# driskai/scenario_gym

Measured on AMD Instinct MI355X. Metric: entity-steps/sec (batched rollout), higher is better.
Workload: dtype f64

## Files before the change

### scenario_gym_amd/csrc/h_queue.hip

```cpp
#include "sgym_host.hpp"

using namespace sgh;

enum { Q_HOST_RING = 16 };
int sgh::check_queue(sg_handle *h)
{
    for (; h->q_count > 0; --h->q_count) {
        const unsigned *w = h->q_host + (size_t)((h->q_head - h->q_count + Q_HOST_RING) % Q_HOST_RING) * sg::Q_STATE_WORDS;
        const unsigned code = w[sg::Q_ERR];
        if (code == 0 || h->q_failed) continue;
        static const char *what[] = {"", "a rollout wavefront waited for the controller pre-pass", "a rollout wavefront waited for the previous chunk of its block",
                                     "the controller pre-pass waited for a buffer of the table ring"};
        h->q_failed = true;
        h->queue_mode = 0;
        snprintf(h->q_msg, sizeof h->q_msg, "sg_rollout: the persistent table launch gave up (%s longer than SG_QUEUE_TIMEOUT_MS; %u work items had finished): "
                                            "the state of the batch is undefined -- sg_reset / sg_upload before the next call", what[code < 4 ? code : 0],
                 w[sg::Q_ITEMS_DONE]);
    }
    return h->q_failed ? fail(h, SG_ERR_HIP, "%s", h->q_msg) : SG_OK;
}
void sgh::forget_queue_failure(sg_handle *h)
{
    h->q_count = 0;
    h->q_failed = false;
// ... 194 lines not shown
}

int sgh::launch_table(sg_handle *h, const LaunchPlan &pl, int n_steps, int force, const double *d_actions, size_t *ev_next)
{
    if (pl.schedule == SCHED_TAB_DUMMY) {
        if (!h->d_tab[0]) {
            HIP_TRY(h, hipMalloc((void **)&h->d_tab[0], 64 * sizeof(double)));
            HIP_TRY(h, hipMalloc((void **)&h->d_tab[1], 64 * sizeof(double)));
            h->tab_bytes = 64 * sizeof(double);
            h->n_tab = 2;
            HIP_TRY(h, hipMemsetAsync(h->d_tab[0], 0, 64 * sizeof(double), h->stream));
        }
        return launch_main(h, pl, pl.fam, n_steps, 0, force, nullptr, h->d_tab[0], ev_next);
    }
    const bool no_overlap = !h->overlap;
    const size_t np = (size_t)h->p.n_ctl_pad, row = (size_t)sg::CT_PLANES * sg::CT_W * np;
    int ch = (int)std::min<size_t>((size_t)std::max(1, h->chunk_steps), std::max<size_t>(1, ((size_t)1 << 27) / row));
    ch = std::min(ch, n_steps);
    if (pl.rss_tab) ch = std::min(ch, std::max(1, h->rssq_steps));
    int rc = SG_QUEUE_FALLBACK;
    if (h->queue_mode && h->WV == 1 && !pl.riders && !no_overlap && np / 64 <= std::min((size_t)h->n_simd, slots_of(h, pl.rss_tab)) / 2 )
        rc = launch_queue(h, n_steps, force, d_actions, ch, ev_next, pl.rss_tab);
    if (rc != SG_QUEUE_FALLBACK) return rc;
    h->last_schedule = 1;
    const int NB = 2;
    const int ctl_slice = h->ctl_slice;
    if (ch > h->p.tab_steps || (size_t)(h->p.tab_steps + 1) * row * sizeof(double) > h->tab_bytes || NB > h->n_tab) {
        const int ts = std::max(ch, h->p.tab_steps);
        const size_t need = (size_t)(ts + 1) * row * sizeof(double);
        if (need > h->tab_bytes || NB > h->n_tab) {
            HIP_TRY(h, hipStreamSynchronize(h->stream));
// ... 27 lines not shown
        n = std::min(std::min(ch, c < 20 ? (2 * h->ctl_slice) << c : ch), n_steps - k0);
        ck0.push_back(k0);
        cn.push_back(n);
    }
    const int C = (int)cn.size();
    std::vector<hipEvent_t> ctl_done((size_t)C, nullptr), chunk_done((size_t)C, nullptr);
    int ctl_issued = 0;
    auto issue_ctl = [&](int upto) -> int {
        for (; ctl_issued <= upto && ctl_issued < C; ++ctl_issued) {
            const int c = ctl_issued, k0 = ck0[(size_t)c], n = cn[(size_t)c];
            double *tab = h->d_tab[c % NB];
            if (!no_overlap && c >= NB)
                HIP_TRY(h, hipStreamWaitEvent(cs, chunk_done[(size_t)(c - NB)], 0));
            for (int s0 = 0; s0 < n; s0 += ctl_slice)
                sgl::control(pl.ctl, cgrid, cs, h->p, h->cfg.timestep, std::min(ctl_slice, n - s0), c == 0 && s0 == 0, k0 + s0, d_actions,
                             tab, s0, pl.ctl_metrics);
            HIP_TRY(h, hipGetLastError());
            if (!no_overlap) {
                const int rc2 = get_event(h, (*ev_next)++, &ctl_done[(size_t)c]);
                if (rc2) return rc2;
                HIP_TRY(h, hipEventRecord(ctl_done[(size_t)c], cs));
            }
        }
        return SG_OK;
    };
    for (int c = 0; c < C; ++c) {
        if ((rc = issue_ctl(std::min(C - 1, c + NB - 1)))) return rc;
        const int b = c % NB;
        const sg::TabGroups tg = one_group(h, h->d_tab[b], cn[(size_t)c]);
        if (!no_overlap) HIP_TRY(h, hipStreamWaitEvent(h->stream, ctl_done[(size_t)c], 0));
        if ((rc = launch_main(h, pl, pl.fam, cn[(size_t)c], 0, force, nullptr, h->d_tab[b], ev_next, &tg))) return rc;
// ... 5 lines not shown
```

### scenario_gym_amd/csrc/h_slice.hip

```cpp
#include "sgym_host.hpp"

using namespace sgh;

static void launch_slice_kernels(sg_handle *h, const Params &ps, const sg::SliceArgs &sa, dim3 grid, const double *tab)
{
    note_slice(h, tab != nullptr);
    sgl::rollout_slice(h->G, grid, h->stream, ps, h->cfg.timestep, sa, tab);
}
static void launch_fixup_kernel(sg_handle *h, const Params &ps, const sg::SliceArgs &sa)
{
    sgl::replay_fixup(h->G, dim3((unsigned)(h->NE / 64)), h->stream, ps, sa, h->d_n_final);
}

struct SlicePlan { int S, len, SG; size_t bytes; };

static SlicePlan slice_plan(const sg_handle *h, int n_steps)
{
    const size_t nblk = h->NE / 64, R = (size_t)h->R, T1 = (size_t)n_steps + 1;
    const bool ctl = h->n_ctl > 0;
    SlicePlan pl{};
    pl.SG = (int)std::max<size_t>(1, 4096 / nblk);
    if (ctl && h->slice_mode == 2) pl.SG = std::min(pl.SG, 8);
    if (!ctl) {
        int S = (int)std::min<size_t>((size_t)pl.SG, (size_t)std::max(1, n_steps / (h->slice_mode == 2 ? 7 : 64)));
// ... 83 lines not shown
        HIP_TRY(h, hipEventRecord(e_reset, h->stream));
        HIP_TRY(h, hipStreamWaitEvent(h->ctl_stream, e_reset, 0));
    }
    HIP_TRY(h, hipMemsetAsync(sa.first_done, 0x7f, (size_t)R * S * sizeof(int), h->stream));
    HIP_TRY(h, hipMemsetAsync(sa.nev, 0, (size_t)R * S * sizeof(int), h->stream));
    const int n_clocks = (int)h->clock_t0.size();
    sgl::clock(dim3((unsigned)((n_clocks + 63) / 64)), h->stream, h->d_clock_t0, n_clocks, h->cfg.timestep, n_steps, const_cast<double *>(sa.tt));
    sa.mode = 0;
    const int ctl_len = std::max(1, env_int("SG_SLICE_CTL_STEPS", 2048));
    for (int s0 = 0; s0 < S; s0 += pl.SG) {
        const int ns = std::min(pl.SG, S - s0);
        if (ctl) {
            const int k0 = s0 * len, k1 = std::min(n_steps, (s0 + ns) * len);
            const dim3 cgrid((unsigned)(ps.n_ctl_pad / 64));
            for (int k = k0; k < k1; k += ctl_len)
                sgl::control(sgl::CTL_FAST, cgrid, h->ctl_stream, ps, h->cfg.timestep, std::min(ctl_len, k1 - k), k == 0, k, nullptr, h->d_slice_tab, k, 0);
            HIP_TRY(h, hipGetLastError());
            hipEvent_t e_c = nullptr;
            if ((rc = get_event(h, ev_next++, &e_c))) return rc;
            HIP_TRY(h, hipEventRecord(e_c, h->ctl_stream));
            HIP_TRY(h, hipStreamWaitEvent(h->stream, e_c, 0));
        }
        hipEvent_t e0 = nullptr, e1 = nullptr;
        if ((rc = get_event(h, ev_next, &e0)) || (rc = get_event(h, ev_next + 1, &e1))) return rc;
        HIP_TRY(h, hipEventRecord(e0, h->stream));
        sa.slice0 = s0;
        launch_slice_kernels(h, ps, sa, dim3((unsigned)nblk, (unsigned)ns), tab);
        HIP_TRY(h, hipGetLastError());
        HIP_TRY(h, hipEventRecord(e1, h->stream));
        h->launch_ev.push_back((int)ev_next);
        ++h->n_launches;
// ... 30 lines not shown
```

### scenario_gym_amd/csrc/k_ctl.hip

```cpp
#define SG_UNIT_CTL
#include "sgym_launch.hpp"

namespace sgl {
void control(int which, dim3 grid, hipStream_t s, const sg::Params &p, double timestep, int n_steps, int first, int k0,
             const double *actions, double *tab, int row0, int metrics)
{
    if (which == CTL_RIDERS) sg::control_kernel_riders<<<grid, dim3(64), 0, s>>>(p, timestep, n_steps, first, k0, actions, tab, row0, metrics);
    else if (which == CTL_FAST) sg::control_kernel_fast<<<grid, dim3(64), 0, s>>>(p, timestep, n_steps, first, k0, actions, tab, row0, metrics);
    else sg::control_kernel<<<grid, dim3(64), 0, s>>>(p, timestep, n_steps, first, k0, actions, tab, row0, metrics);
}
}
```

### scenario_gym_amd/csrc/sgym_control.hpp

```cpp
#pragma once

namespace sg {

struct CtlLds { double ctrl[9][64]; double seg[5][64]; };

template <bool FAST, bool RIDERS = false>
__device__ __forceinline__ void control_body_l(CtlLds &lds ,
                                               const unsigned qblock ,
                                               const Params &p, double timestep, int n_steps, int first, int k0,
                                               const double *actions , double *tab, int row0, int metrics)
{
    const int lane = threadIdx.x;
    const size_t q = (size_t)qblock * 64 + lane;
    const int ent_raw = p.ctl_ent[q];
    const bool active = ent_raw >= 0;
    const uint32_t ent = active ? (uint32_t)ent_raw : 0u;
    const uint32_t r = ent / (uint32_t)p.EP;
    const LanePtr st(p.stat + (size_t)(ent >> 6) * (ST_COUNT * 64), (ent & 63) * 8u);
    const LanePtr dy(p.dyn + (size_t)(ent >> 6) * ((size_t)p.FROWS * 64), (ent & 63) * 8u);
    const int64_t meta = fld<int64_t>(st, ST_META);
    const int kind = active ? (int)(meta & 0xff) : SG_KIND_NONE;
    const double min_t = fld(st, ST_MIN_T), bl = fld(st, ST_BL);
    const bool is_ego = active && (int)(ent - r * (uint32_t)p.EP) == p.sstat[r].ego;
#pragma unroll
    for (int c = 0; c < 9; ++c) lds.ctrl[c][lane] = fld(st, ST_CTRL + c);
    const size_t NP = (size_t)p.n_ctl_pad;
    double *cst = p.ctl_state + q;

    double pose[6], t, prev_t;
    double m_avg, m_max, m_t;
    bool present;
    CtrlState cs;
    if (first) {
        const sg_scenario_state &sd = p.sdyn[r];
        t = sd.t;
        prev_t = sd.prev_t;
        m_avg = sd.ego_avg_speed; m_max = sd.ego_max_speed; m_t = sd.avg_t;
        present = fld<uint64_t>(dy, SG_F_PRESENT) != 0;
#pragma unroll
        for (int c = 0; c < 6; ++c) pose[c] = fld(dy, SG_F_POSE + c);
        cs.speed = fld(dy, SG_F_CTRL + 0); cs.e_lon_prev = fld(dy, SG_F_CTRL + 1);
        cs.e_lat_prev = fld(dy, SG_F_CTRL + 2); cs.e_lon_int = fld(dy, SG_F_CTRL + 3);
    } else {
#pragma unroll
        for (int c = 0; c < 6; ++c) pose[c] = cst[(CS_POSE + c) * NP];
        present = cst[CS_PRESENT * NP] != 0.0;
        cs.speed = cst[(CS_CTRL + 0) * NP]; cs.e_lon_prev = cst[(CS_CTRL + 1) * NP];
        cs.e_lat_prev = cst[(CS_CTRL + 2) * NP]; cs.e_lon_int = cst[(CS_CTRL + 3) * NP];
        t = cst[CS_T * NP];
        prev_t = cst[CS_PREV_T * NP];
        m_avg = cst[(CS_METRIC + 0) * NP]; m_max = cst[(CS_METRIC + 1) * NP]; m_t = cst[(CS_METRIC + 2) * NP];
    }
    if (!active) present = false;

    Table T;
    {
        const double *kn = p.knots + fld<int64_t>(st, ST_KNOT_OFF) * 7;
        T.x = kn; T.xs = 7; T.y = kn + 1; T.ys = 7; T.cs = 1;
        T.n = active ? (int)(meta >> 32) : 0;
    }
    double seg_hi;
    int seg_cur;
    double sgr[5] = {0.0, 0.0, 0.0, 0.0, 0.0};
    auto seg_publish = [&](const Segment &S) {
        lds.seg[0][lane] = S.x_lo;
        lds.seg[1][lane] = S.ylo[0]; lds.seg[2][lane] = S.ylo[1];
// ... 63 lines not shown
            steer = __builtin_fmin(__builtin_fmax(steer, -max_steer), max_steer);
            const double dxs = speed0 * cos_h, dys = speed0 * sin_h;
            double tan_s = sg_tan_poly(steer, K);
            const bool steep = !(__builtin_fabs(steer) < 0.67434);
            if (sg_any(steep & active)) {
                double s2, c2;
                sg_sincos_core(steer, s2, c2, K);
                tan_s = steep ? s2 / c2 : tan_s;
            }
            const double hnum = speed0 * tan_s;
            const double dh = hnum == 0.0 ? hnum : rd_l.div(hnum);
            const double nx = pose[0] + dxs * dt, ny = pose[1] + dys * dt, nh = pose[3] + dh * dt;
            double nspeed = speed0 + accel * dt;
            nspeed = allow_rev == 0.0 ? __builtin_fmax(0.0, nspeed) : nspeed;
            nspeed = max_speed == max_speed ? __builtin_fmin(max_speed, nspeed) : nspeed;
            bool ok = rd.safe(d_lat) & rd.safe(d_lon) & (__builtin_fabs(steer) < 1.0e5) & (rd_l.safe(hnum) | (hnum == 0.0));
            double n_avg = m_avg, n_max = m_max, n_mt = m_t;
            if (metrics) {
                const RecipDiv rdt(dt), rnt(next_t);
                const double ax = nx - pose[0], ay = ny - pose[1];
                const double az = pose[2] - pose[2];
                const double speed = sg_norm3(rdt.div(ax), rdt.div(ay), 0.0);
                const double w = rnt.div(m_t);
                n_avg = m_avg + (1.0 - w) * (speed - m_avg);
                n_max = __builtin_fmax(speed, m_max);
                n_mt = next_t;
                ok = ok & (!is_ego | (rdt.safe(ax) & rdt.safe(ay) & rnt.safe(m_t) & (dt > 0.0) & (az == 0.0)));
            }
            if (sg_all(!active || ok)) {
                cs.e_lat_prev = e_lat; cs.e_lon_prev = e_lon; cs.e_lon_int = e_lon_I; cs.speed = nspeed;
                pose[0] = nx; pose[1] = ny; pose[3] = nh;
                if (is_ego) { m_avg = n_avg; m_max = n_max; m_t = n_mt; }
                prev_t = t;
                t = next_t;
                *reinterpret_cast<double4 *>(out + (size_t)k * CT_W) = make_double4(pose[0], pose[1], pose[3], cs.speed);
                *reinterpret_cast<double4 *>(out1 + (size_t)k * CT_W) = make_double4(cs.e_lon_prev, cs.e_lat_prev, cs.e_lon_int, 0.0);
                if (is_ego && metrics) *reinterpret_cast<double4 *>(out2 + (size_t)k * CT_W) = make_double4(m_avg, m_max, m_t, 0.0);
                continue;
            }
        }
        double act_a = 0.0, act_s = 0.0;
        if (kind == SG_KIND_AGENT_VEHICLE && actions) {
            const double *a = actions + ((size_t)(k0 + k) * p.R + r) * 2;
            act_a = a[0];
            act_s = a[1];
        }
        if (next_t > seg_hi) {
            Segment S;
            S.x_hi = seg_hi;
            S.cur = seg_cur;
            seg_advance(T, S, next_t);
            seg_publish(S);
// ... 21 lines not shown
            auto cp = [&](int q) -> double { return lds.ctrl[q][lane]; };
            if (kind == SG_KIND_AGENT_PID)
                pid_step(cs, cp, bl, state_dt, dt, tx, ty, sin_h, cos_h, np_, K);
            else
                vehicle_step(cs, cp, bl, dt, act_a, act_s, sin_h, cos_h, np_, K);
        } else if (active && min_t >= t) {
            npres = true;
            Segment S;
            S.cur = seg_cur;
            seg_load(T, S);
            sg_loads_done();
            const double dqs = next_t - S.x_lo;
#pragma unroll
            for (int c = 0; c < 6; ++c) np_[c] = S.sl[c] * dqs + S.ylo[c];
        }
        if (is_ego && npres && metrics) {
            double prev[6];
            if (!present) {
                own_position_extrap(T.x, T.n, t, prev);
                sg_loads_done();
            } else {
#pragma unroll
                for (int c = 0; c < 6; ++c) prev[c] = pose[c];
            }
            const double v0 = (np_[0] - prev[0]) / dt, v1 = (np_[1] - prev[1]) / dt, v2 = (np_[2] - prev[2]) / dt;
            const double speed = sg_norm3(v0, v1, v2);
            const double w = m_t / next_t;
            m_avg += (1.0 - w) * (speed - m_avg);
            m_t = next_t;
            m_max = __builtin_fmax(speed, m_max);
        }
        present = npres;
        if (npres) {
#pragma unroll
            for (int c = 0; c < 6; ++c) pose[c] = np_[c];
        }
        prev_t = t;
        t = next_t;
        *reinterpret_cast<double4 *>(out + (size_t)k * CT_W) = make_double4(pose[0], pose[1], pose[3], cs.speed);
        *reinterpret_cast<double4 *>(out1 + (size_t)k * CT_W) = make_double4(cs.e_lon_prev, cs.e_lat_prev, cs.e_lon_int, 0.0);
        if (is_ego && metrics) *reinterpret_cast<double4 *>(out2 + (size_t)k * CT_W) = make_double4(m_avg, m_max, m_t, 0.0);
        if (RIDERS) *reinterpret_cast<double4 *>(out2 + (size_t)k * CT_W) = make_double4(pose[2], pose[4], pose[5], present ? 1.0 : 0.0);
    }
#pragma unroll
    for (int c = 0; c < 6; ++c) cst[(CS_POSE + c) * NP] = pose[c];
    cst[CS_PRESENT * NP] = present ? 1.0 : 0.0;
    cst[(CS_CTRL + 0) * NP] = cs.speed; cst[(CS_CTRL + 1) * NP] = cs.e_lon_prev;
    cst[(CS_CTRL + 2) * NP] = cs.e_lat_prev; cst[(CS_CTRL + 3) * NP] = cs.e_lon_int;
    cst[CS_T * NP] = t;
    cst[CS_PREV_T * NP] = prev_t;
    cst[(CS_METRIC + 0) * NP] = m_avg; cst[(CS_METRIC + 1) * NP] = m_max; cst[(CS_METRIC + 2) * NP] = m_t;
}

template <bool FAST, bool RIDERS = false>
__device__ __forceinline__ void control_body(const Params &p, double timestep, int n_steps, int first, int k0,
                                             const double *actions , double *tab, int row0, int metrics)
{
    __shared__ CtlLds lds;
    control_body_l<FAST, RIDERS>(lds, blockIdx.x, p, timestep, n_steps, first, k0, actions, tab, row0, metrics);
}

#ifdef SG_UNIT_CTL
static __global__ __launch_bounds__(64, SG_CTL_WAVES) void control_kernel(Params p, double timestep, int n_steps, int first, int k0,
                                                     const double *actions , double *tab, int row0, int metrics)
{
    control_body<false>(p, timestep, n_steps, first, k0, actions, tab, row0, metrics);
}
#endif
#ifdef SG_UNIT_CTL
static __global__ __launch_bounds__(64, 2) void control_kernel_riders(Params p, double timestep, int n_steps, int first, int k0,
                                                               const double *actions , double *tab, int row0, int metrics)
{
    control_body<false, true>(p, timestep, n_steps, first, k0, actions, tab, row0, 0);
}
#endif
#ifdef SG_UNIT_CTL
static __global__ __launch_bounds__(64, 1) void control_kernel_fast(Params p, double timestep, int n_steps, int first, int k0,
                                                             const double *actions , double *tab, int row0, int metrics)
{
#ifdef SG_CTL_SETPRIO
    __builtin_amdgcn_s_setprio(3);
#endif
    control_body<true>(p, timestep, n_steps, first, k0, actions, tab, row0, metrics);
}
#endif

}
```

### scenario_gym_amd/csrc/sgym_core.hpp

```cpp
#pragma once

namespace sg {

enum {
    ST_BW = 0, ST_BL, ST_BCX, ST_BCY,
    ST_MIN_T, ST_MAX_T,
    ST_KNOT_OFF,
    ST_META,
    ST_ROUTE,
    ST_CTL,
    ST_CTRL,
    NCTRL_ROWS = 13,
    ST_COUNT = ST_CTRL + NCTRL_ROWS
};
constexpr uint32_t ROW = 512;

struct ScenStatic {
    double t0, length;
    int64_t grid_off;
    int32_t grid_n, ego;
};

struct RoadNet { double x0, y0, inv_cell; int32_t nx, ny; int64_t cell_base; };
struct RoadCand { int32_t poly; uint32_t edge_off; uint16_t n_edges; uint8_t ref_sel, ref_inside; };
// ... 54 lines not shown
    const double *noise_normals;
    long long noise_len;
    unsigned long long noise_seed;
    int ped_behaviour;
    int n_ped_models;
    const double *ped_models;
    const int32_t *model_of;
#ifdef SG_PHASE_TIMERS
    unsigned long long *phase_cycles;
#endif
};

enum { PM_BEHAVIOUR = 0, PM_SF = 1, PM_STD_LON = 13, PM_STD_LAT = 14, PM_W = 16 };
static_assert(sizeof(sg_social_force) == 12 * sizeof(double), "sg_social_force is twelve doubles");

enum { CT_X = 0, CT_Y, CT_H, CT_SPEED, CT_W = 4, CT_ELON = 0, CT_ELAT, CT_EINT, CT_MAVG = 0, CT_MMAX, CT_MT, CT_PLANES = 3 };
enum { CS_POSE = 0, CS_PRESENT = 6, CS_CTRL = 7, CS_T = 11, CS_PREV_T = 12, CS_METRIC = 13, CS_COUNT = 16 };

#define SG_GLOBAL __attribute__((address_space(1)))
struct LanePtr {
    SG_GLOBAL char *a[3];
    __device__ __forceinline__ LanePtr(const double *blk, uint32_t voff)
    {
        a[0] = (SG_GLOBAL char *)(reinterpret_cast<char *>(const_cast<double *>(blk)) + voff);
        a[1] = a[0] + 8 * ROW;
        a[2] = a[0] + 16 * ROW;
        asm("" : "+v"(a[1]), "+v"(a[2]));
    }
};
template <typename T = double>
__device__ __forceinline__ T fld(const LanePtr &lp, int f)
{
// ... 344 lines not shown
```

### scenario_gym_amd/csrc/sgym_hip.hip

```cpp
#include "sgym_host.hpp"

using namespace sgh;

static void note_kernel(sg_handle *h, const char *fmt, int a = 0, int b = 0) { snprintf(h->last_kernel, sizeof h->last_kernel, fmt, a, b); }
void sgh::note_wide(sg_handle *h) { note_kernel(h, "sg::wide_move_kernel + wide_commit_kernel + wide_collide_kernel + wide_finish_kernel"); }
void sgh::note_queue(sg_handle *h, bool rss)
{
    note_kernel(h, rss ? "sg::rollout_kernel_rss_tabq<%d>" : (h->planar ? "sg::rollout_kernel_tabq_planar<%d>" : "sg::rollout_kernel_tabq<%d>"), h->G);
}
void sgh::note_slice(sg_handle *h, bool tab) { note_kernel(h, tab ? "sg::rollout_kernel_slice_tab<%d>" : "sg::rollout_kernel_slice<%d>", h->G); }

static Fam pick_family(const sg_handle *h, bool rss, bool tab)
{
    const bool ped = h->has_ped, off_road = (h->cfg.terminal_mask & SG_TERM_EGO_OFF_ROAD) != 0;
    if (h->WV == 8) {
        if (!ped && off_road) return Fam::ROAD_W8;
        if (rss && !ped) return Fam::RSS_W8;
        return ped ? Fam::PED_W8 : Fam::PLAIN_W8;
    }
    if (ped && h->all_ped && h->G == 64 && crowd_road_ok(h) && crowd_allowed(h) && !rss) return Fam::CROWD;
    if (tab && ped && h->G == 64) return Fam::CROWD_RIDERS;
    if (ped && rss) return Fam::RSS_PED;
    if (rss && off_road) return Fam::RSS_ROAD;
    if (ped) return Fam::PED;
// ... 93 lines not shown
        pl.schedule = SCHED_STEPWISE;
        pl.reset_fam = pl.fam = pick_family(h, pl.rss_lines, false);
        return pl;
    }
    pl.riders = allow_tab && h->crowd_riders && crowd_road_ok(h) && !rss && h->n_ctl > 0 && n_steps >= h->tab_min;
    pl.rss_tab = allow_tab && rss && h->WV == 1 && !h->has_ped && !off_road && h->n_ext == 0 && h->n_ctl > 0 && n_steps >= h->tab_min &&
                 env_int("SG_RSS_TAB", 1) != 0;
    const bool use_tab = pl.riders || pl.rss_tab || (allow_tab && h->WV <= 4 && !h->has_ped && !rss && !off_road && h->n_ext == 0 &&
                                                     n_steps >= h->tab_min && h->max_ctl_per_block <= SG_TAB_LANES(h->G, h->WV));
    pl.timed = use_tab || n_steps >= 16;
    pl.reset_fam = pick_family(h, rss, false);
    pl.fam = pick_family(h, rss, use_tab);
    pl.schedule = !use_tab ? SCHED_ONE : h->n_ctl == 0 ? SCHED_TAB_DUMMY : SCHED_TAB;
    if (pl.riders) pl.ctl = sgl::CTL_RIDERS;
    else if (pl.rss_tab && env_int("SG_RSS_CTL_FAST", 1) != 0) pl.ctl = sgl::CTL_FAST;
    pl.ctl_metrics = pl.riders || pl.rss_tab ? 0 : 1;
    return pl;
}

int sgh::launch_plan(sg_handle *h, const LaunchPlan &pl, int n_steps, int do_reset, int force, const double *d_actions)
{
    h->n_launches = 0;
    h->launch_ev.clear();
    if (pl.timed) HIP_TRY(h, hipEventRecord(h->ev0, h->stream));
    size_t ev_next = 0;
    int rc = SG_OK;
    switch (pl.schedule) {
    case SCHED_WIDE:
        rc = launch_wide(h, n_steps, do_reset, force, d_actions, pl.rss_alone);
        break;
    case SCHED_STEPWISE:
// ... 136 lines not shown
```

### scenario_gym_amd/csrc/sgym_host.hpp

```cpp
#pragma once
#include <hip/hip_runtime.h>

#include <algorithm>
#include <functional>
#include <atomic>
#include <cassert>
#include <cmath>
#include <cstdarg>
#include <cstdio>
#include <cstdlib>
#include <chrono>
#include <cstring>
#include <iterator>
#include <memory>
#include <string>
#include <thread>
#include <vector>

#include "sgym_launch.hpp"

using sg::Params;

namespace sgh {

// ... 349 lines not shown
{
    return dim3((unsigned)std::min<size_t>(h->NE / 64, (size_t)tg.len0 + tg.len1));
}

enum class Fam { ROAD_W8, RSS_W8, PED_W8, PLAIN_W8, CROWD, CROWD_RIDERS, RSS_PED, RSS_ROAD, PED, RSS_TAB, RSS, ROAD, TAB, TAB_ROWS, PLAIN };

enum Schedule { SCHED_WIDE, SCHED_STEPWISE, SCHED_ONE, SCHED_TAB_DUMMY, SCHED_TAB };
struct LaunchPlan {
    Schedule schedule = SCHED_ONE;
    Fam reset_fam = Fam::PLAIN;
    Fam fam = Fam::PLAIN;
    bool rss_lines = false;
    bool rss_alone = false;
    bool off_road = false;
    bool riders = false, rss_tab = false;
    int ctl = sgl::CTL_GENERAL, ctl_metrics = 1;
    bool timed = false;
};

LaunchPlan plan_call(const sg_handle *h, int n_steps, bool rss, bool allow_tab);
int launch_plan(sg_handle *h, const LaunchPlan &pl, int n_steps, int do_reset, int force, const double *d_actions);
int launch_rollout(sg_handle *h, int n_steps, int do_reset, int force, const double *d_actions, bool rss = false);
int launch_main(sg_handle *h, const LaunchPlan &pl, Fam fam, int n_steps, int do_reset, int force, const double *d_actions,
                const double *d_tab, size_t *ev_next, const sg::TabGroups *groups = nullptr);
int rss_fused_call(sg_handle *h, bool live_only, bool *fused, bool *fresh = nullptr);
int get_event(sg_handle *h, size_t idx, hipEvent_t *out);
int ensure_actions(sg_handle *h, size_t n, bool *grew = nullptr);
int step_forced(sg_handle *h, int n_steps, const double *d_actions);
void note_wide(sg_handle *h);
void note_queue(sg_handle *h, bool rss);
void note_slice(sg_handle *h, bool tab);
// ... 77 lines not shown
```

### scenario_gym_amd/csrc/sgym_launch.hpp

```cpp
#pragma once
#include "sgym_device.hpp"
#include "sgym_wide.hpp"
#include "sgym_queue.hpp"
#include "sgym_policy.hpp"
#include "sgym_episode.hpp"

namespace sgl {

struct RolloutArgs {
    const sg::Params *p;
    double timestep;
    int n_steps, do_reset, force;
    const double *actions;
    const double *tab;
};

void rollout_plain(int G, int WV, bool tab, dim3 grid, hipStream_t s, const RolloutArgs &a);
void rollout_ped(int G, int WV, bool rss, dim3 grid, hipStream_t s, const RolloutArgs &a);
void rollout_ped_rss(int G, int WV, dim3 grid, hipStream_t s, const RolloutArgs &a);
void rollout_crowd(int WV, bool riders, dim3 grid, hipStream_t s, const RolloutArgs &a, bool models = false);
void wide_step(dim3 grid_entities, dim3 grid_scenarios, hipStream_t s, const sg::Params &p, double timestep, const sg::WideArgs &wa,
               bool no_peds );
void wide_running(hipStream_t s, const sg::Params &p, int *host_word);
void rollout_rss(int G, int WV, bool road, dim3 grid, hipStream_t s, const RolloutArgs &a);
// ... 20 lines not shown
                       int n_ahead, double spacing, double *feat, int32_t *info);
void drive(hipStream_t s, const sg::Params &p, double timestep, const int32_t *scen, const int32_t *slot, int64_t n, const double *actions,
           double *ext);
void driver_policy(hipStream_t s, const sg::Params &p, const sg::PolicyIndex &P, const int32_t *scen, const int32_t *slot, int64_t m,
                   const int32_t *row_of, double *actions, int32_t *info, double *feat);
void episode(hipStream_t s, const sg::EpisodeArgs &a);
void episode_clear(hipStream_t s, const uint8_t *mask, const sg::EpisodeArgs &a);
void rollout_tab(int G, bool planar, dim3 grid, hipStream_t s, const sg::Params &p, double timestep, int force, const sg::TabGroups &tg);
void rollout_tabq(int G, bool planar, dim3 grid, hipStream_t s, const sg::Params &p, double timestep, int force, const sg::TabQueue &tq);
int tabq_waves_per_cu(int G, bool planar);
int rss_tabq_waves_per_cu(int G);
void rollout_rss_tabq(int G, dim3 grid, hipStream_t s, const sg::Params &p, double timestep, int force, const sg::TabQueue &tq);
void rollout_slice(int G, dim3 grid, hipStream_t s, const sg::Params &p, double timestep, const sg::SliceArgs &sa, const double *tab);
enum { CTL_GENERAL = 0, CTL_RIDERS = 1, CTL_FAST = 2 };
void control(int which, dim3 grid, hipStream_t s, const sg::Params &p, double timestep, int n_steps, int first, int k0,
             const double *actions, double *tab, int row0, int metrics);
void event_ego_pose(dim3 grid, hipStream_t s, const sg::Params &p, const sg::TabGroups &tg);
void terminal_flags(dim3 grid, hipStream_t s, const sg::Params &p, double timestep, uint32_t *out);
void classify_events(dim3 grid, hipStream_t s, const sg::Params &p, double c_tol);
void rss(dim3 grid, dim3 block, hipStream_t s, const sg::Params &p, int reset, int32_t *rss_state, int32_t *code, double *safe, int32_t *seen);
void ego_off_road(dim3 grid, hipStream_t s, const sg::Params &p);
void replay_fixup(int G, dim3 grid, hipStream_t s, const sg::Params &p, const sg::SliceArgs &sa, const int *n_final);
void replay_scenario_fixup(dim3 grid, hipStream_t s, const sg::Params &p, const sg::SliceArgs &sa, const int *n_final, const int *done_in);
void slice_final(dim3 grid, hipStream_t s, const sg::Params &p, const sg::SliceArgs &sa, int *n_final, int *done_out);
void clock(dim3 grid, hipStream_t s, const double *t0, int n_clocks, double timestep, int n_total, double *tt);
void delay(hipStream_t s, long long ticks);
void build_grid(dim3 grid, hipStream_t s, const sg::Params &p, const int32_t *row_scen, int64_t row0, int64_t row_end);
void trig32(dim3 grid, hipStream_t s, const double *h, float *sin_out, float *cos_out, int64_t n);

}

// ... 24 lines not shown
```

### scenario_gym_amd/csrc/sgym_queue.hpp

```cpp
#pragma once

namespace sg {

enum { Q_TICKET = 0, Q_HEAD = 1, Q_ERR = 2, Q_ITEMS_DONE = 3, Q_CTL_CLAIMED = 4, Q_STATE_WORDS = 8 };
constexpr int Q_SEATS = 1 << 14;
enum { Q_ERR_CTL_WAIT = 1, Q_ERR_BLOCK_WAIT = 2, Q_ERR_RING_WAIT = 3 };
constexpr int Q_MAX_CHUNKS = 255;
constexpr int Q_PROG_STRIDE = 32;

struct TabQueue {
    unsigned *state;
    unsigned *ctl_prog;
    unsigned *blk_prog;
    unsigned *chunk_cnt;
    unsigned *seats;
    long long defer_ticks;
    double *tab;
    size_t buf_doubles;
    const double *actions;
    unsigned *trace;
    unsigned long long *times;
    long long timeout_ticks;
    int n_chunks, n_buf, nblk, n_ctl_waves;
    int nap;
// ... 95 lines not shown
        }
        if (claim) {
            unsigned idx = 0;
            if (lane == 0) idx = atomicAdd(tq.state + Q_CTL_CLAIMED, 1u);
            idx = (unsigned)__builtin_amdgcn_readfirstlane((int)idx);
            if (idx < (unsigned)tq.n_ctl_waves) ticket = idx;
        }
    }

    if (ticket < (unsigned)tq.n_ctl_waves) {
        __builtin_amdgcn_s_setprio(3);
        CtlLds &cl = *reinterpret_cast<CtlLds *>(&lds);
        for (int c = 0; c < tq.n_chunks; ++c) {
            if (c >= tq.n_buf && !q_wait_ge(tq.chunk_cnt + (c - tq.n_buf), (unsigned)tq.nblk, tq, Q_ERR_RING_WAIT)) break;
            control_body_l<true>(cl, ticket, p, timestep, tq.k0[c + 1] - tq.k0[c], c == 0, tq.k0[c], tq.actions,
                                 tq.tab + (size_t)(c % tq.n_buf) * tq.buf_doubles, 0, RSS ? 0 : 1);
            q_release();
            if (tq.times && lane == 0) tq.times[(size_t)tq.n_chunks * tq.nblk * 4 + (size_t)ticket * tq.n_chunks + c] = wall_clock64();
            if (lane == 0) __hip_atomic_store(tq.ctl_prog + ticket * Q_PROG_STRIDE, (unsigned)(c + 1), __ATOMIC_RELAXED, __HIP_MEMORY_SCOPE_AGENT);
        }
        __builtin_amdgcn_s_setprio(0);
        if (q_peek(tq.state + Q_ERR) != 0) return;
    }

    const unsigned n_items = (unsigned)tq.n_chunks * (unsigned)tq.nblk;
    unsigned done_b = ~0u, done_c = 0;
    for (;;) {
        unsigned item = 0;
        if (lane == 0) {
            if (done_b != ~0u) {
                __hip_atomic_store(tq.blk_prog + done_b, done_c + 1, __ATOMIC_RELAXED, __HIP_MEMORY_SCOPE_AGENT);
// ... 119 lines not shown
```

### scenario_gym_amd/csrc/sgym_rollout.hpp

```cpp
#pragma once

namespace sg {

enum : unsigned {
    V_PED = 1,
    V_TAB = 2,
    V_HAST = 4,
    V_ROAD = 8,
    V_RSS = 16,
    V_CROWD = 32,
    V_SLICE = 64,
    V_PLANAR = 128,
    V_RIDERS = 256,
    V_CTAB = 512,
    V_MODELS = 1024
};

template <int G, int WV, unsigned F>
struct Variant {
    static constexpr bool PED = (F & V_PED) != 0, TAB = (F & V_TAB) != 0, HAST = (F & V_HAST) != 0, ROAD = (F & V_ROAD) != 0,
                          RSSV = (F & V_RSS) != 0, CROWD = (F & V_CROWD) != 0, SLICE = (F & V_SLICE) != 0, PLANAR = (F & V_PLANAR) != 0,
                          RIDERS = (F & V_RIDERS) != 0, CTAB = (F & V_CTAB) != 0, MODELS = !CROWD || (F & V_MODELS) != 0;
    static_assert(F < 2 * V_MODELS, "flags: V_* bits only");
    static_assert(!SLICE || (TAB && WV == 1 && !PED && !ROAD && !RSSV), "slices: the table variant, one wavefront per tile");
// ... 33 lines not shown

struct SliceArgs {
    int mode;
    int n_slices, len;
    int n_total;
    const double *tt;
    const int *clock_of;
    double *dnorm;
    double2 *espeed;
    int *first_done;
    sg_event *ev;
    int *nev;
    const int *n_final;
    int slice0;
};

template <int G, int WV, unsigned F>
__device__ __forceinline__ void rollout_body_l(
    typename Variant<G, WV, F>::Lds &lds ,
    const Params &p, double timestep, int n_steps, int do_reset, int force, const double *actions ,
    const double *tab , const SliceArgs &sa = SliceArgs{},
    const unsigned bx_arg = ~0u )
{
    const unsigned bx = bx_arg == ~0u ? blockIdx.x : bx_arg;
    using V = Variant<G, WV, F>;
    constexpr bool PED = V::PED, TAB = V::TAB, ROAD = V::ROAD, RSSV = V::RSSV, CROWD = V::CROWD, SLICE = V::SLICE, PLANAR = V::PLANAR,
                   RIDERS = V::RIDERS, CTAB = V::CTAB, MODELS = V::MODELS;
    constexpr bool HAS_TAB = V::HAS_TAB, REFINE = V::REFINE, LATE = V::LATE, PARK = V::PARK;
    constexpr int NS = V::NS, TL = V::TL;
    const int tid = threadIdx.x, lane = tid & 63, wave = tid >> 6;
// ... 966 lines not shown
            else {
#pragma unroll
                for (int w = 0; w < WV; ++w) (w < 4 ? sd.last_row[w & 3] : sd.last_row_hi[w & 3]) = last_row[w];
            }
        }
        if (HAS_TAB && sa.mode == 1 && in_range && tab_lane) {
            const double *lr = tab + (size_t)ctl_q * tab_lane_stride + (size_t)(sa.n_final[r] - 1) * CT_W;
            const double *lr1 = lr + (size_t)p.n_ctl_pad * tab_lane_stride;
            stf(dy, SG_F_CTRL + 0, lr[CT_SPEED]); stf(dy, SG_F_CTRL + 1, lr1[CT_ELON]);
            stf(dy, SG_F_CTRL + 2, lr1[CT_ELAT]); stf(dy, SG_F_CTRL + 3, lr1[CT_EINT]);
        }
        return;
    }
    ego_fetch();
    if (RSSV && lane == 0) p.rssq_n[rss_wave] = min(rss_gn, p.rssq_cap);
    if (in_range) {
        const LanePtr dx = dy_again();
        sg_scenario_state &sx = sd_again();
        if (PED && kind == SG_KIND_AGENT_PEDESTRIAN) cs.e_lon_prev = (double)goal_idx;
        if (LATE) {
            stf(dx, SG_F_POSE + 0, pose[0]); stf(dx, SG_F_POSE + 1, pose[1]); stf(dx, SG_F_POSE + 3, pose[3]);
            if (!PLANAR) { stf(dx, SG_F_POSE + 2, pose[2]); stf(dx, SG_F_POSE + 4, pose[4]); stf(dx, SG_F_POSE + 5, pose[5]); }
            stf(dx, SG_F_DIST, dist);
            stf(dx, SG_F_PRESENT, (uint64_t)present);
#pragma unroll
            for (int w = 0; w < WV; ++w) stf(dx, SG_F_COLL + w, row[w]);
        }
        if (TAB) {
            if (tab_lane && last_k >= 0) {
                const int64_t ctl_x = fld<int64_t>(rows_again(st), ST_CTL);
                const double *lr = tab + (size_t)ctl_x * tab_lane_stride + (size_t)last_k * CT_W;
                const double *lr1 = lr + (size_t)p.n_ctl_pad * tab_lane_stride;
                stf(dx, SG_F_CTRL + 0, lr[CT_SPEED]); stf(dx, SG_F_CTRL + 1, lr1[CT_ELON]);
                stf(dx, SG_F_CTRL + 2, lr1[CT_ELAT]); stf(dx, SG_F_CTRL + 3, lr1[CT_EINT]);
                if (is_ego) {
                    const double *lr2 = lr1 + (size_t)p.n_ctl_pad * tab_lane_stride;
                    m_avg = lr2[CT_MAVG]; m_max = lr2[CT_MMAX]; m_t = lr2[CT_MT];
                }
            }
        } else if ((RIDERS || CTAB) && rider) {
            if (last_k >= 0 && (kind == SG_KIND_AGENT_PID || kind == SG_KIND_AGENT_VEHICLE)) {
                const double *lr = rider_row + (size_t)last_k * CT_W;
                const double *lr1 = lr + (size_t)p.n_ctl_pad * tab_lane_stride;
                stf(dx, SG_F_CTRL + 0, lr[CT_SPEED]); stf(dx, SG_F_CTRL + 1, lr1[CT_ELON]);
                stf(dx, SG_F_CTRL + 2, lr1[CT_ELAT]); stf(dx, SG_F_CTRL + 3, lr1[CT_EINT]);
            }
        } else {
            stf(dx, SG_F_CTRL + 0, cs.speed); stf(dx, SG_F_CTRL + 1, cs.e_lon_prev);
            stf(dx, SG_F_CTRL + 2, cs.e_lat_prev); stf(dx, SG_F_CTRL + 3, cs.e_lon_int);
        }
        if (slot == 0) { sx.t = t; sx.prev_t = prev_t; sx.done = done; sx.n_steps = steps; if (PED) sx.noise_pos = noise_pos; }
        if (RSSV) {
            if (slot < p.E) {
// ... 223 lines not shown
        }
    }
}

#ifdef SG_UNIT_MAIN
static __global__ __launch_bounds__(64) void replay_scenario_fixup_kernel(Params p, SliceArgs sa, const int *n_final, const int *done_in)
{
    const int lane = threadIdx.x;
    const int r = (int)blockIdx.x * 64 + lane;
    if (r >= p.R) return;
    sg_scenario_state &sd = p.sdyn[r];
    const int nf = n_final[r];
    double m_avg = sd.ego_avg_speed, m_max = sd.ego_max_speed, m_t = sd.avg_t;
    const double2 *es = sa.espeed + r;
    const double *tr = sa.tt + (size_t)sa.clock_of[r] * (size_t)(sa.n_total + 1);
    auto update = [&](double2 e, double t, bool divide) {
        const bool valid = e.x == e.x;
        double c = e.y;
        if (divide) c = (c != c) ? 1.0 - m_t / t : c;
        const double a = m_avg + c * (e.x - m_avg);
        m_avg = valid ? a : m_avg;
        m_t = valid ? t : m_t;
        m_max = valid ? __builtin_fmax(e.x, m_max) : m_max;
    };
    constexpr int NB = 16;
    double2 spa[NB], spb[NB];
    double tqa[NB], tqb[NB];
    auto fetch = [&](double2 (&sp)[NB], double (&tq)[NB], int q0) {
#pragma unroll
        for (int u = 0; u < NB; ++u) {
            const int qq = min(q0 + u, sa.n_total);
            sp[u] = es[(size_t)qq * p.R];
            tq[u] = tr[qq];
        }
    };
    auto work = [&](const double2 (&sp)[NB], const double (&tq)[NB]) {
        bool need = false;
#pragma unroll
        for (int u = 0; u < NB; ++u) need |= (sp[u].x == sp[u].x) & (sp[u].y != sp[u].y);
// ... 37 lines not shown
```

Measured before the change: 148.9 billion.

## Move ego speed metrics from controller pre-pass into rollout wave-parallel pass

The controller pre-pass no longer tracks the ego average, max speed and clock per step, and it stops writing the third table plane. It now stores the clock in the second plane instead. The rollout kernel rebuilds the metrics afterwards with a wave-cooperative pass: lanes compute per-step speeds and blend coefficients in parallel into LDS, then the ego lane runs the serial average recurrence. This shortens the serial controller critical path and shrinks the table buffer, at the cost of extra rollout work, LDS traffic and possible floating-point rounding differences.

After: 154.5 billion, median of 6. 1.04x the previous value.

```diff
diff --git a/scenario_gym_amd/csrc/h_queue.hip b/scenario_gym_amd/csrc/h_queue.hip
--- a/scenario_gym_amd/csrc/h_queue.hip
+++ b/scenario_gym_amd/csrc/h_queue.hip
@@ -232,7 +232,7 @@
         return launch_main(h, pl, pl.fam, n_steps, 0, force, nullptr, h->d_tab[0], ev_next);
     }
     const bool no_overlap = !h->overlap;
-    const size_t np = (size_t)h->p.n_ctl_pad, row = (size_t)sg::CT_PLANES * sg::CT_W * np;
+    const size_t np = (size_t)h->p.n_ctl_pad, row = (size_t)(pl.riders ? sg::CT_PLANES_RIDERS : sg::CT_PLANES) * sg::CT_W * np;
     int ch = (int)std::min<size_t>((size_t)std::max(1, h->chunk_steps), std::max<size_t>(1, ((size_t)1 << 27) / row));
     ch = std::min(ch, n_steps);
     if (pl.rss_tab) ch = std::min(ch, std::max(1, h->rssq_steps));
@@ -290,7 +290,7 @@
                 HIP_TRY(h, hipStreamWaitEvent(cs, chunk_done[(size_t)(c - NB)], 0));
             for (int s0 = 0; s0 < n; s0 += ctl_slice)
                 sgl::control(pl.ctl, cgrid, cs, h->p, h->cfg.timestep, std::min(ctl_slice, n - s0), c == 0 && s0 == 0, k0 + s0, d_actions,
-                             tab, s0, pl.ctl_metrics);
+                             tab, s0);
             HIP_TRY(h, hipGetLastError());
             if (!no_overlap) {
                 const int rc2 = get_event(h, (*ev_next)++, &ctl_done[(size_t)c]);
diff --git a/scenario_gym_amd/csrc/h_slice.hip b/scenario_gym_amd/csrc/h_slice.hip
--- a/scenario_gym_amd/csrc/h_slice.hip
+++ b/scenario_gym_amd/csrc/h_slice.hip
@@ -121,7 +121,7 @@
             const int k0 = s0 * len, k1 = std::min(n_steps, (s0 + ns) * len);
             const dim3 cgrid((unsigned)(ps.n_ctl_pad / 64));
             for (int k = k0; k < k1; k += ctl_len)
-                sgl::control(sgl::CTL_FAST, cgrid, h->ctl_stream, ps, h->cfg.timestep, std::min(ctl_len, k1 - k), k == 0, k, nullptr, h->d_slice_tab, k, 0);
+                sgl::control(sgl::CTL_FAST, cgrid, h->ctl_stream, ps, h->cfg.timestep, std::min(ctl_len, k1 - k), k == 0, k, nullptr, h->d_slice_tab, k);
             HIP_TRY(h, hipGetLastError());
             hipEvent_t e_c = nullptr;
             if ((rc = get_event(h, ev_next++, &e_c))) return rc;
diff --git a/scenario_gym_amd/csrc/k_ctl.hip b/scenario_gym_amd/csrc/k_ctl.hip
--- a/scenario_gym_amd/csrc/k_ctl.hip
+++ b/scenario_gym_amd/csrc/k_ctl.hip
@@ -3,10 +3,10 @@
 
 namespace sgl {
 void control(int which, dim3 grid, hipStream_t s, const sg::Params &p, double timestep, int n_steps, int first, int k0,
-             const double *actions, double *tab, int row0, int metrics)
+             const double *actions, double *tab, int row0)
 {
-    if (which == CTL_RIDERS) sg::control_kernel_riders<<<grid, dim3(64), 0, s>>>(p, timestep, n_steps, first, k0, actions, tab, row0, metrics);
-    else if (which == CTL_FAST) sg::control_kernel_fast<<<grid, dim3(64), 0, s>>>(p, timestep, n_steps, first, k0, actions, tab, row0, metrics);
-    else sg::control_kernel<<<grid, dim3(64), 0, s>>>(p, timestep, n_steps, first, k0, actions, tab, row0, metrics);
+    if (which == CTL_RIDERS) sg::control_kernel_riders<<<grid, dim3(64), 0, s>>>(p, timestep, n_steps, first, k0, actions, tab, row0);
+    else if (which == CTL_FAST) sg::control_kernel_fast<<<grid, dim3(64), 0, s>>>(p, timestep, n_steps, first, k0, actions, tab, row0);
+    else sg::control_kernel<<<grid, dim3(64), 0, s>>>(p, timestep, n_steps, first, k0, actions, tab, row0);
 }
 }
diff --git a/scenario_gym_amd/csrc/sgym_control.hpp b/scenario_gym_amd/csrc/sgym_control.hpp
--- a/scenario_gym_amd/csrc/sgym_control.hpp
+++ b/scenario_gym_amd/csrc/sgym_control.hpp
@@ -8,7 +8,7 @@
 __device__ __forceinline__ void control_body_l(CtlLds &lds ,
                                                const unsigned qblock ,
                                                const Params &p, double timestep, int n_steps, int first, int k0,
-                                               const double *actions , double *tab, int row0, int metrics)
+                                               const double *actions , double *tab, int row0)
 {
     const int lane = threadIdx.x;
     const size_t q = (size_t)qblock * 64 + lane;
@@ -21,21 +21,18 @@
     const int64_t meta = fld<int64_t>(st, ST_META);
     const int kind = active ? (int)(meta & 0xff) : SG_KIND_NONE;
     const double min_t = fld(st, ST_MIN_T), bl = fld(st, ST_BL);
-    const bool is_ego = active && (int)(ent - r * (uint32_t)p.EP) == p.sstat[r].ego;
 #pragma unroll
     for (int c = 0; c < 9; ++c) lds.ctrl[c][lane] = fld(st, ST_CTRL + c);
     const size_t NP = (size_t)p.n_ctl_pad;
     double *cst = p.ctl_state + q;
 
     double pose[6], t, prev_t;
-    double m_avg, m_max, m_t;
     bool present;
     CtrlState cs;
     if (first) {
         const sg_scenario_state &sd = p.sdyn[r];
         t = sd.t;
         prev_t = sd.prev_t;
-        m_avg = sd.ego_avg_speed; m_max = sd.ego_max_speed; m_t = sd.avg_t;
         present = fld<uint64_t>(dy, SG_F_PRESENT) != 0;
 #pragma unroll
         for (int c = 0; c < 6; ++c) pose[c] = fld(dy, SG_F_POSE + c);
@@ -49,7 +46,6 @@
         cs.e_lat_prev = cst[(CS_CTRL + 2) * NP]; cs.e_lon_int = cst[(CS_CTRL + 3) * NP];
         t = cst[CS_T * NP];
         prev_t = cst[CS_PREV_T * NP];
-        m_avg = cst[(CS_METRIC + 0) * NP]; m_max = cst[(CS_METRIC + 1) * NP]; m_t = cst[(CS_METRIC + 2) * NP];
     }
     if (!active) present = false;
 
@@ -143,28 +139,14 @@
             double nspeed = speed0 + accel * dt;
             nspeed = allow_rev == 0.0 ? __builtin_fmax(0.0, nspeed) : nspeed;
             nspeed = max_speed == max_speed ? __builtin_fmin(max_speed, nspeed) : nspeed;
-            bool ok = rd.safe(d_lat) & rd.safe(d_lon) & (__builtin_fabs(steer) < 1.0e5) & (rd_l.safe(hnum) | (hnum == 0.0));
-            double n_avg = m_avg, n_max = m_max, n_mt = m_t;
-            if (metrics) {
-                const RecipDiv rdt(dt), rnt(next_t);
-                const double ax = nx - pose[0], ay = ny - pose[1];
-                const double az = pose[2] - pose[2];
-                const double speed = sg_norm3(rdt.div(ax), rdt.div(ay), 0.0);
-                const double w = rnt.div(m_t);
-                n_avg = m_avg + (1.0 - w) * (speed - m_avg);
-                n_max = __builtin_fmax(speed, m_max);
-                n_mt = next_t;
-                ok = ok & (!is_ego | (rdt.safe(ax) & rdt.safe(ay) & rnt.safe(m_t) & (dt > 0.0) & (az == 0.0)));
-            }
+            const bool ok = rd.safe(d_lat) & rd.safe(d_lon) & (__builtin_fabs(steer) < 1.0e5) & (rd_l.safe(hnum) | (hnum == 0.0));
             if (sg_all(!active || ok)) {
                 cs.e_lat_prev = e_lat; cs.e_lon_prev = e_lon; cs.e_lon_int = e_lon_I; cs.speed = nspeed;
                 pose[0] = nx; pose[1] = ny; pose[3] = nh;
-                if (is_ego) { m_avg = n_avg; m_max = n_max; m_t = n_mt; }
                 prev_t = t;
                 t = next_t;
                 *reinterpret_cast<double4 *>(out + (size_t)k * CT_W) = make_double4(pose[0], pose[1], pose[3], cs.speed);
-                *reinterpret_cast<double4 *>(out1 + (size_t)k * CT_W) = make_double4(cs.e_lon_prev, cs.e_lat_prev, cs.e_lon_int, 0.0);
-                if (is_ego && metrics) *reinterpret_cast<double4 *>(out2 + (size_t)k * CT_W) = make_double4(m_avg, m_max, m_t, 0.0);
+                *reinterpret_cast<double4 *>(out1 + (size_t)k * CT_W) = make_double4(cs.e_lon_prev, cs.e_lat_prev, cs.e_lon_int, t);
                 continue;
             }
         }
@@ -216,22 +198,6 @@
 #pragma unroll
             for (int c = 0; c < 6; ++c) np_[c] = S.sl[c] * dqs + S.ylo[c];
         }
-        if (is_ego && npres && metrics) {
-            double prev[6];
-            if (!present) {
-                own_position_extrap(T.x, T.n, t, prev);
-                sg_loads_done();
-            } else {
-#pragma unroll
-                for (int c = 0; c < 6; ++c) prev[c] = pose[c];
-            }
-            const double v0 = (np_[0] - prev[0]) / dt, v1 = (np_[1] - prev[1]) / dt, v2 = (np_[2] - prev[2]) / dt;
-            const double speed = sg_norm3(v0, v1, v2);
-            const double w = m_t / next_t;
-            m_avg += (1.0 - w) * (speed - m_avg);
-            m_t = next_t;
-            m_max = __builtin_fmax(speed, m_max);
-        }
         present = npres;
         if (npres) {
 #pragma unroll
@@ -240,8 +206,7 @@
         prev_t = t;
         t = next_t;
         *reinterpret_cast<double4 *>(out + (size_t)k * CT_W) = make_double4(pose[0], pose[1], pose[3], cs.speed);
-        *reinterpret_cast<double4 *>(out1 + (size_t)k * CT_W) = make_double4(cs.e_lon_prev, cs.e_lat_prev, cs.e_lon_int, 0.0);
-        if (is_ego && metrics) *reinterpret_cast<double4 *>(out2 + (size_t)k * CT_W) = make_double4(m_avg, m_max, m_t, 0.0);
+        *reinterpret_cast<double4 *>(out1 + (size_t)k * CT_W) = make_double4(cs.e_lon_prev, cs.e_lat_prev, cs.e_lon_int, t);
         if (RIDERS) *reinterpret_cast<double4 *>(out2 + (size_t)k * CT_W) = make_double4(pose[2], pose[4], pose[5], present ? 1.0 : 0.0);
     }
 #pragma unroll
@@ -251,40 +216,39 @@
     cst[(CS_CTRL + 2) * NP] = cs.e_lat_prev; cst[(CS_CTRL + 3) * NP] = cs.e_lon_int;
     cst[CS_T * NP] = t;
     cst[CS_PREV_T * NP] = prev_t;
-    cst[(CS_METRIC + 0) * NP] = m_avg; cst[(CS_METRIC + 1) * NP] = m_max; cst[(CS_METRIC + 2) * NP] = m_t;
 }
 
 template <bool FAST, bool RIDERS = false>
 __device__ __forceinline__ void control_body(const Params &p, double timestep, int n_steps, int first, int k0,
-                                             const double *actions , double *tab, int row0, int metrics)
+                                             const double *actions , double *tab, int row0)
 {
     __shared__ CtlLds lds;
-    control_body_l<FAST, RIDERS>(lds, blockIdx.x, p, timestep, n_steps, first, k0, actions, tab, row0, metrics);
+    control_body_l<FAST, RIDERS>(lds, blockIdx.x, p, timestep, n_steps, first, k0, actions, tab, row0);
 }
 
 #ifdef SG_UNIT_CTL
 static __global__ __launch_bounds__(64, SG_CTL_WAVES) void control_kernel(Params p, double timestep, int n_steps, int first, int k0,
-                                                     const double *actions , double *tab, int row0, int metrics)
-{
-    control_body<false>(p, timestep, n_steps, first, k0, actions, tab, row0, metrics);
+                                                     const double *actions , double *tab, int row0)
+{
+    control_body<false>(p, timestep, n_steps, first, k0, actions, tab, row0);
 }
 #endif
 #ifdef SG_UNIT_CTL
 static __global__ __launch_bounds__(64, 2) void control_kernel_riders(Params p, double timestep, int n_steps, int first, int k0,
-                                                               const double *actions , double *tab, int row0, int metrics)
-{
-    control_body<false, true>(p, timestep, n_steps, first, k0, actions, tab, row0, 0);
+                                                               const double *actions , double *tab, int row0)
+{
+    control_body<false, true>(p, timestep, n_steps, first, k0, actions, tab, row0);
 }
 #endif
 #ifdef SG_UNIT_CTL
 static __global__ __launch_bounds__(64, 1) void control_kernel_fast(Params p, double timestep, int n_steps, int first, int k0,
-                                                             const double *actions , double *tab, int row0, int metrics)
+                                                             const double *actions , double *tab, int row0)
 {
 #ifdef SG_CTL_SETPRIO
     __builtin_amdgcn_s_setprio(3);
 #endif
-    control_body<true>(p, timestep, n_steps, first, k0, actions, tab, row0, metrics);
-}
-#endif
-
-}
+    control_body<true>(p, timestep, n_steps, first, k0, actions, tab, row0);
+}
+#endif
+
+}
diff --git a/scenario_gym_amd/csrc/sgym_core.hpp b/scenario_gym_amd/csrc/sgym_core.hpp
--- a/scenario_gym_amd/csrc/sgym_core.hpp
+++ b/scenario_gym_amd/csrc/sgym_core.hpp
@@ -92,8 +92,8 @@
 enum { PM_BEHAVIOUR = 0, PM_SF = 1, PM_STD_LON = 13, PM_STD_LAT = 14, PM_W = 16 };
 static_assert(sizeof(sg_social_force) == 12 * sizeof(double), "sg_social_force is twelve doubles");
 
-enum { CT_X = 0, CT_Y, CT_H, CT_SPEED, CT_W = 4, CT_ELON = 0, CT_ELAT, CT_EINT, CT_MAVG = 0, CT_MMAX, CT_MT, CT_PLANES = 3 };
-enum { CS_POSE = 0, CS_PRESENT = 6, CS_CTRL = 7, CS_T = 11, CS_PREV_T = 12, CS_METRIC = 13, CS_COUNT = 16 };
+enum { CT_X = 0, CT_Y, CT_H, CT_SPEED, CT_W = 4, CT_ELON = 0, CT_ELAT, CT_EINT, CT_T, CT_PLANES = 2, CT_PLANES_RIDERS = 3 };
+enum { CS_POSE = 0, CS_PRESENT = 6, CS_CTRL = 7, CS_T = 11, CS_PREV_T = 12, CS_COUNT = 13 };
 
 #define SG_GLOBAL __attribute__((address_space(1)))
 struct LanePtr {
diff --git a/scenario_gym_amd/csrc/sgym_hip.hip b/scenario_gym_amd/csrc/sgym_hip.hip
--- a/scenario_gym_amd/csrc/sgym_hip.hip
+++ b/scenario_gym_amd/csrc/sgym_hip.hip
@@ -131,7 +131,6 @@
     pl.schedule = !use_tab ? SCHED_ONE : h->n_ctl == 0 ? SCHED_TAB_DUMMY : SCHED_TAB;
     if (pl.riders) pl.ctl = sgl::CTL_RIDERS;
     else if (pl.rss_tab && env_int("SG_RSS_CTL_FAST", 1) != 0) pl.ctl = sgl::CTL_FAST;
-    pl.ctl_metrics = pl.riders || pl.rss_tab ? 0 : 1;
     return pl;
 }
 
diff --git a/scenario_gym_amd/csrc/sgym_host.hpp b/scenario_gym_amd/csrc/sgym_host.hpp
--- a/scenario_gym_amd/csrc/sgym_host.hpp
+++ b/scenario_gym_amd/csrc/sgym_host.hpp
@@ -387,7 +387,7 @@
     bool rss_alone = false;
     bool off_road = false;
     bool riders = false, rss_tab = false;
-    int ctl = sgl::CTL_GENERAL, ctl_metrics = 1;
+    int ctl = sgl::CTL_GENERAL;
     bool timed = false;
 };
 
diff --git a/scenario_gym_amd/csrc/sgym_launch.hpp b/scenario_gym_amd/csrc/sgym_launch.hpp
--- a/scenario_gym_amd/csrc/sgym_launch.hpp
+++ b/scenario_gym_amd/csrc/sgym_launch.hpp
@@ -58,7 +58,7 @@
 void rollout_slice(int G, dim3 grid, hipStream_t s, const sg::Params &p, double timestep, const sg::SliceArgs &sa, const double *tab);
 enum { CTL_GENERAL = 0, CTL_RIDERS = 1, CTL_FAST = 2 };
 void control(int which, dim3 grid, hipStream_t s, const sg::Params &p, double timestep, int n_steps, int first, int k0,
-             const double *actions, double *tab, int row0, int metrics);
+             const double *actions, double *tab, int row0);
 void event_ego_pose(dim3 grid, hipStream_t s, const sg::Params &p, const sg::TabGroups &tg);
 void terminal_flags(dim3 grid, hipStream_t s, const sg::Params &p, double timestep, uint32_t *out);
 void classify_events(dim3 grid, hipStream_t s, const sg::Params &p, double c_tol);
diff --git a/scenario_gym_amd/csrc/sgym_queue.hpp b/scenario_gym_amd/csrc/sgym_queue.hpp
--- a/scenario_gym_amd/csrc/sgym_queue.hpp
+++ b/scenario_gym_amd/csrc/sgym_queue.hpp
@@ -133,7 +133,7 @@
         for (int c = 0; c < tq.n_chunks; ++c) {
             if (c >= tq.n_buf && !q_wait_ge(tq.chunk_cnt + (c - tq.n_buf), (unsigned)tq.nblk, tq, Q_ERR_RING_WAIT)) break;
             control_body_l<true>(cl, ticket, p, timestep, tq.k0[c + 1] - tq.k0[c], c == 0, tq.k0[c], tq.actions,
-                                 tq.tab + (size_t)(c % tq.n_buf) * tq.buf_doubles, 0, RSS ? 0 : 1);
+                                 tq.tab + (size_t)(c % tq.n_buf) * tq.buf_doubles, 0);
             q_release();
             if (tq.times && lane == 0) tq.times[(size_t)tq.n_chunks * tq.nblk * 4 + (size_t)ticket * tq.n_chunks + c] = wall_clock64();
             if (lane == 0) __hip_atomic_store(tq.ctl_prog + ticket * Q_PROG_STRIDE, (unsigned)(c + 1), __ATOMIC_RELAXED, __HIP_MEMORY_SCOPE_AGENT);
diff --git a/scenario_gym_amd/csrc/sgym_rollout.hpp b/scenario_gym_amd/csrc/sgym_rollout.hpp
--- a/scenario_gym_amd/csrc/sgym_rollout.hpp
+++ b/scenario_gym_amd/csrc/sgym_rollout.hpp
@@ -71,6 +71,92 @@
     const int *n_final;
     int slice0;
 };
+
+__device__ __forceinline__ void ego_avg_step(double &m_avg, double speed, double c) { m_avg = m_avg + c * (speed - m_avg); }
+__device__ __forceinline__ void ego_speed_step(double &m_avg, double &m_max, double speed, double c)
+{
+    ego_avg_step(m_avg, speed, c);
+    m_max = __builtin_fmax(speed, m_max);
+}
+__device__ __forceinline__ void ego_speed_update(double &m_avg, double &m_max, double &m_t, double2 e, double t, bool divide)
+{
+    const bool valid = e.x == e.x;
+    double c = e.y;
+    if (divide) c = (c != c) ? 1.0 - m_t / t : c;
+    double a = m_avg, mx = m_max;
+    ego_speed_step(a, mx, e.x, c);
+    m_avg = valid ? a : m_avg;
+    m_t = valid ? t : m_t;
+    m_max = valid ? mx : m_max;
+}
+
+template <int GL, bool PLANAR>
+__device__ __forceinline__ void ego_metric_pass(double *lds_speed, double *lds_c , const int lane,
+                                                const int tile0, const bool ego_do, const int n, const double *col ,
+                                                const size_t plane1 , const double px0,
+                                                const double py0, const double dz0, const double dzr, const double t_start,
+                                                double &m_avg, double &m_max, const double m_t)
+{
+    const uint64_t em = __ballot(ego_do);
+    if (em == 0) return;
+    uint64_t tm = em >> tile0;
+    if (GL < 64) tm &= (1ull << (GL & 63)) - 1;
+    const bool has = tm != 0;
+    const int el = has ? tile0 + (int)__builtin_ctzll(tm) : lane;
+    const int n_t = has ? __shfl(n, el, 64) : 0;
+    const uint64_t col_bits = __shfl((unsigned long long)(uintptr_t)col, el, 64);
+    const double *colp = reinterpret_cast<const double *>((uintptr_t)col_bits);
+    const double dzr_t = PLANAR ? 0.0 : shfl_d(dzr, el);
+    const int j = (lane - el) & (GL - 1);
+    double *const my_speed = lds_speed + tile0, *const my_c = lds_c + tile0;
+    double2 a1 = make_double2(0.0, 0.0), a0 = a1;
+    double t1 = 0.0, t0 = 0.0;
+    auto fetch = [&](int k) {
+        if (k < n_t) {
+            const double *r1 = colp + (size_t)k * CT_W, *r0 = r1 - (k > 0 ? CT_W : 0);
+            a1 = *reinterpret_cast<const double2 *>(r1);
+            a0 = *reinterpret_cast<const double2 *>(r0);
+            t1 = r1[plane1 + CT_T];
+            t0 = r0[plane1 + CT_T];
+        }
+    };
+    fetch(j);
+    double lmax = __builtin_nan("");
+    for (int base = 0; sg_any(base < n_t); base += GL) {
+        const int k = base + j;
+        if (k < n_t) {
+            const bool head = k == 0;
+            const double px = head ? px0 : a0.x, py = head ? py0 : a0.y, tp = head ? t_start : t0;
+            const double mt = head ? m_t : t0;
+            const double dt = t1 - tp;
+            const double v2 = PLANAR ? 0.0 : (head ? dz0 : dzr_t) / dt;
+            const double speed = sg_norm3((a1.x - px) / dt, (a1.y - py) / dt, v2);
+            lmax = __builtin_fmax(speed, lmax);
+            my_speed[j] = speed;
+            my_c[j] = 1.0 - mt / t1;
+        }
+        fetch(k + GL);
+        __builtin_amdgcn_wave_barrier();
+        asm volatile("" ::: "memory");
+        if (ego_do) {
+            const int cnt = min(GL, n - base);
+            int u = 0;
+            for (; u + 8 <= cnt; u += 8) {
+                double sp[8], cc[8];
+#pragma unroll
+                for (int q = 0; q < 8; ++q) { sp[q] = my_speed[u + q]; cc[q] = my_c[u + q]; }
+#pragma unroll
+                for (int q = 0; q < 8; ++q) ego_avg_step(m_avg, sp[q], cc[q]);
+            }
+            for (; u < cnt; ++u) ego_avg_step(m_avg, my_speed[u], my_c[u]);
+        }
+        __builtin_amdgcn_wave_barrier();
+        asm volatile("" ::: "memory");
+    }
+#pragma unroll
+    for (int o = 1; o < GL; o <<= 1) lmax = __builtin_fmax(lmax, shfl_d(lmax, lane ^ o));
+    if (ego_do) m_max = __builtin_fmax(lmax, m_max);
+}
 
 template <int G, int WV, unsigned F>
 __device__ __forceinline__ void rollout_body_l(
@@ -1067,6 +1153,31 @@
     }
     ego_fetch();
     if (RSSV && lane == 0) p.rssq_n[rss_wave] = min(rss_gn, p.rssq_cap);
+    if (HAS_TAB) {
+        static_assert(!HAS_TAB || LATE || SLICE, "the pass reads the rows and the record's clock the item began with: nothing may have stored them yet");
+        const bool ego_do = in_range && is_ego && tab_lane && last_k >= 0 && present;
+        double px0 = 0.0, py0 = 0.0, dz0 = 0.0, dzr = 0.0, t_start = 0.0;
+        const double *col = tab;
+        if (ego_do) {
+            const LanePtr d0 = dy_again(), st_o = rows_again(st);
+            col = tab + (size_t)fld<int64_t>(st_o, ST_CTL) * tab_lane_stride;
+            t_start = sd_again().t;
+            px0 = fld(d0, SG_F_POSE + 0);
+            py0 = fld(d0, SG_F_POSE + 1);
+            if (!PLANAR) dzr = dz0 = pose[2] - pose[2];
+            if (fld<uint64_t>(d0, SG_F_PRESENT) == 0) {
+                double prev[6];
+                own_position_extrap(p.knots + fld<int64_t>(st_o, ST_KNOT_OFF) * 7, (int)(fld<int64_t>(st_o, ST_META) >> 32), t_start, prev);
+                px0 = prev[0];
+                py0 = prev[1];
+                if (!PLANAR) dz0 = pose[2] - prev[2];
+            }
+            sg_loads_done();
+        }
+        ego_metric_pass<(WV == 1 ? G : 64), PLANAR>(&lds.ctrl[3][sl - lane], &lds.ctrl[4][sl - lane], lane, tile0, ego_do, last_k + 1, col,
+                                                    (size_t)p.n_ctl_pad * tab_lane_stride, px0, py0, dz0, dzr, t_start, m_avg, m_max, m_t);
+        if (ego_do) m_t = t;
+    }
     if (in_range) {
         const LanePtr dx = dy_again();
         sg_scenario_state &sx = sd_again();
@@ -1086,10 +1197,6 @@
                 const double *lr1 = lr + (size_t)p.n_ctl_pad * tab_lane_stride;
                 stf(dx, SG_F_CTRL + 0, lr[CT_SPEED]); stf(dx, SG_F_CTRL + 1, lr1[CT_ELON]);
                 stf(dx, SG_F_CTRL + 2, lr1[CT_ELAT]); stf(dx, SG_F_CTRL + 3, lr1[CT_EINT]);
-                if (is_ego) {
-                    const double *lr2 = lr1 + (size_t)p.n_ctl_pad * tab_lane_stride;
-                    m_avg = lr2[CT_MAVG]; m_max = lr2[CT_MMAX]; m_t = lr2[CT_MT];
-                }
             }
         } else if ((RIDERS || CTAB) && rider) {
             if (last_k >= 0 && (kind == SG_KIND_AGENT_PID || kind == SG_KIND_AGENT_VEHICLE)) {
@@ -1343,15 +1450,7 @@
     double m_avg = sd.ego_avg_speed, m_max = sd.ego_max_speed, m_t = sd.avg_t;
     const double2 *es = sa.espeed + r;
     const double *tr = sa.tt + (size_t)sa.clock_of[r] * (size_t)(sa.n_total + 1);
-    auto update = [&](double2 e, double t, bool divide) {
-        const bool valid = e.x == e.x;
-        double c = e.y;
-        if (divide) c = (c != c) ? 1.0 - m_t / t : c;
-        const double a = m_avg + c * (e.x - m_avg);
-        m_avg = valid ? a : m_avg;
-        m_t = valid ? t : m_t;
-        m_max = valid ? __builtin_fmax(e.x, m_max) : m_max;
-    };
+    auto update = [&](double2 e, double t, bool divide) { ego_speed_update(m_avg, m_max, m_t, e, t, divide); };
     constexpr int NB = 16;
     double2 spa[NB], spb[NB];
     double tqa[NB], tqb[NB];
```
